# kkromberg/SpeechRecognition

Measured on AMD Instinct MI355X. Metric: frames/sec scored+decoded, higher is better.
Workload: dtype f64

## Files before the change

### include/srgpu.h

```cpp
#ifndef SRGPU_H
#define SRGPU_H

#include <stddef.h>
#include <stdint.h>

#ifdef __cplusplus
extern "C" {
#endif

#if defined(__GNUC__)
#define SR_API __attribute__((visibility("default")))
#else
#define SR_API
#endif

#define SR_ABI_VERSION 4
SR_API int sr_abi_version(void);

#define SR_OK 0
#define SR_EINVAL (-1)
#define SR_EHIP (-2)
#define SR_ENODEV (-3)
#define SR_ELIMIT (-4)
#define SR_ENOMEM (-5)
// ... 252 lines not shown
SR_API int sr_bigram_word_lattice_corpus(sr_model* m, sr_corpus* c, sr_bigram* b, int gmm_kernel, double lattice_beam, uint64_t cap,
                                         uint64_t* out_arc_off, double* out_best, uint32_t* out_word, uint32_t* out_hist,
                                         uint32_t* out_pred, uint32_t* out_first, uint32_t* out_last, double* out_fwd, double* out_bwd,
                                         double* out_am);
SR_API int sr_bigram_lattice_nbest(uint32_t n_frames, uint64_t n_arcs, const uint32_t* word, const uint32_t* hist,
                                   const uint32_t* first, const uint32_t* last, const double* am, uint32_t n_words,
                                   uint32_t silence_word, const float* lm, double lm_scale, uint32_t n_best, uint32_t* out_words,
                                   uint64_t words_cap, uint64_t* out_off, double* out_cost, uint32_t* out_count);

typedef struct sr_bigram_stream sr_bigram_stream;
SR_API int sr_bigram_stream_open(sr_model* m, sr_bigram* b, const sr_bigram_params* p, uint32_t max_streams, uint64_t max_frames,
                                 sr_bigram_stream** out);
SR_API int sr_bigram_stream_begin(sr_bigram_stream* s, uint32_t* id);
SR_API int sr_bigram_stream_push(sr_bigram_stream* s, uint32_t n, const uint32_t* ids, const float* feats, const uint64_t* frame_off);
SR_API int sr_bigram_stream_partial(sr_bigram_stream* s, uint32_t id, uint32_t* out_word, float* out_score, uint32_t* out_time,
                                    uint32_t cap, uint32_t* count, uint64_t* frames);
SR_API int sr_bigram_stream_end(sr_bigram_stream* s, uint32_t id, uint32_t* out_word, float* out_score, uint32_t* out_time,
                                uint32_t cap, uint32_t* count);
SR_API int sr_bigram_stream_destroy(sr_bigram_stream* s);

SR_API int sr_probe_fp16_denormals(int device, int* preserved);
SR_API int sr_probe_fp16_accumulation(int device, int* within_model, double* worst_ratio);

typedef struct {
  double gmm_ms;
  uint64_t gmm_launches;
  double gmm_flops;
  double search_ms;
  uint64_t search_launches;
  double search_bytes;
  uint64_t frames;
  uint64_t refined_pairs;
  uint64_t refined_densities;
  double prefilter_ms;
  double refine_ms;
} sr_profile;
SR_API int sr_profile_enable(sr_model* m, int on);
SR_API int sr_profile_reset(sr_model* m);
SR_API int sr_profile_read(sr_model* m, sr_profile* out);

#ifdef __cplusplus
}
#endif
#endif
```

### speechrecognition_amd/capi.py

```python
from __future__ import annotations

import ctypes as C
import os

import numpy as np

HERE = os.path.dirname(os.path.abspath(__file__))
LIB_PATH = os.environ.get("SRGPU_LIB") or os.path.join(HERE, "libsrgpu.so")

GMM_MFMA, GMM_EXACT, GMM_PREFILTER, GMM_DEFAULT = 0, 1, 2, 3
POOL_GLOBAL, POOL_MIXTURE, POOL_NONE = 0, 1, 2
SEARCH_GENERAL_KERNEL = 1
SEARCH_SLOT_KERNEL = 2
BIGRAM_DENSE_STATES = 1
BIGRAM_GLOBAL_STATES = 2
SR_ECORRUPT = -7
LDA_SKIP = 0xFFFFFFFF
SR_ABI_VERSION = 4

SYMBOLS = [
    "sr_abi_version", "sr_model_trim",
    "sr_last_error", "sr_device_count", "sr_model_create", "sr_model_load_mixset", "sr_model_destroy", "sr_model_info",
    "sr_corpus_upload", "sr_corpus_upload_async", "sr_corpus_wait", "sr_corpus_destroy", "sr_shard_utterances", "sr_recognize_batch_multi", "sr_score_corpus", "sr_score_frames", "sr_lexicon_create",
    "sr_lexicon_destroy", "sr_lexicon_describe", "sr_recognize_corpus", "sr_traceback_corpus", "sr_traceback_words", "sr_recognize_batch", "sr_align_corpus", "sr_align_corpus_pruned", "sr_path_scores_corpus", "sr_model_create_from_statistics", "sr_model_create_from_accumulated", "sr_mixset_write", "sr_model_set_tying", "sr_model_tying_info", "sr_model_topology", "sr_accumulate_corpus",
    "sr_model_split", "sr_model_eliminate", "sr_model_tables",
    "sr_state_posteriors_corpus", "sr_baum_welch_corpus", "sr_word_posteriors_corpus", "sr_recognize_confidence_corpus",
    "sr_net_occupancies_corpus", "sr_mmi_statistics_corpus", "sr_model_create_from_mmi_statistics",
    "sr_smbr_max_positions", "sr_net_accuracies_corpus", "sr_smbr_statistics_corpus",
    "sr_word_lattice_corpus", "sr_lattice_nbest",
    "sr_fmllr_statistics_corpus", "sr_fmllr_statistics_bw_corpus", "sr_fmllr_estimate", "sr_corpus_transform",
    "sr_mllr_statistics_corpus", "sr_mllr_statistics_bw_corpus", "sr_mllr_estimate", "sr_model_transform_means",
    "sr_mllt_statistics_corpus", "sr_mllt_statistics_bw_corpus", "sr_mllt_estimate",
    "sr_lda_statistics_corpus", "sr_lda_estimate", "sr_corpus_splice_transform",
    "sr_bigram_create", "sr_bigram_destroy", "sr_bigram_describe", "sr_recognize_bigram_corpus",
    "sr_bigram_word_posteriors_corpus", "sr_recognize_bigram_confidence_corpus",
    "sr_bigram_occupancies_corpus", "sr_bigram_mmi_statistics_corpus",
    "sr_bigram_accuracies_corpus", "sr_bigram_smbr_statistics_corpus",
    "sr_bigram_word_lattice_corpus", "sr_bigram_lattice_nbest",
    "sr_stream_open", "sr_stream_begin", "sr_stream_push", "sr_stream_partial", "sr_stream_end", "sr_stream_destroy",
    "sr_bigram_stream_open", "sr_bigram_stream_begin", "sr_bigram_stream_push", "sr_bigram_stream_partial", "sr_bigram_stream_end",
    "sr_bigram_stream_destroy",
    "sr_probe_fp16_denormals", "sr_probe_fp16_accumulation",
    "sr_profile_enable", "sr_profile_reset", "sr_profile_read",
]


class SrError(RuntimeError):
    def __init__(self, code, msg):
        super().__init__(f"libsrgpu error {code}: {msg}")
        self.code = code


def smbr_max_positions():
    n = C.c_uint32()
    _check(lib().sr_smbr_max_positions(C.byref(n)))
    return n.value


class SearchParams(C.Structure):
    _fields_ = [("am_threshold", C.c_double), ("word_penalty", C.c_double), ("gmm_kernel", C.c_int), ("flags", C.c_int)]


class BigramParams(C.Structure):
    _fields_ = [("acoustic_pruning", C.c_float), ("lm_pruning", C.c_float), ("gmm_kernel", C.c_int), ("max_word_ends", C.c_uint32), ("flags", C.c_int)]


class Profile(C.Structure):
    _fields_ = [("gmm_ms", C.c_double), ("gmm_launches", C.c_uint64), ("gmm_flops", C.c_double),
                ("search_ms", C.c_double), ("search_launches", C.c_uint64), ("search_bytes", C.c_double),
                ("frames", C.c_uint64), ("refined_pairs", C.c_uint64), ("refined_densities", C.c_uint64),
                ("prefilter_ms", C.c_double), ("refine_ms", C.c_double)]


# ... 77 lines not shown
        L.sr_recognize_bigram_corpus.argtypes = [vp, vp, vp, C.POINTER(BigramParams), vp, vp, vp, vp]
        L.sr_bigram_word_posteriors_corpus.argtypes = [vp, vp, vp, i32, dbl, dbl, u32, vp, vp, vp, vp]
        L.sr_bigram_occupancies_corpus.argtypes = [vp, vp, vp, i32, dbl, dbl, u32, vp, vp, vp, vp, vp, vp]
        L.sr_bigram_mmi_statistics_corpus.argtypes = [vp, vp, vp, i32, dbl, dbl, i32, vp, vp] + [vp] * 10
        L.sr_bigram_accuracies_corpus.argtypes = [vp, vp, vp, i32, dbl, dbl, u32, vp, vp, vp, vp, vp, vp]
        L.sr_bigram_smbr_statistics_corpus.argtypes = [vp, vp, vp, i32, dbl, dbl, i32, vp] + [vp] * 10
        L.sr_recognize_bigram_confidence_corpus.argtypes = [vp, vp, vp, C.POINTER(BigramParams), dbl, vp, vp, vp, vp, vp]
        L.sr_bigram_word_lattice_corpus.argtypes = [vp, vp, vp, i32, dbl, u64] + [vp] * 10
        L.sr_bigram_lattice_nbest.argtypes = [u32, u64, vp, vp, vp, vp, vp, u32, u32, vp, dbl, u32, vp, u64, vp, vp, C.POINTER(u32)]
        L.sr_stream_open.argtypes = [vp, vp, C.POINTER(SearchParams), u32, u64, C.POINTER(vp)]
        L.sr_stream_begin.argtypes = [vp, C.POINTER(u32)]
        L.sr_stream_push.argtypes = [vp, u32, vp, vp, vp]
        L.sr_stream_partial.argtypes = [vp, u32, vp, u32, C.POINTER(u32), C.POINTER(u64)]
        L.sr_stream_end.argtypes = [vp, u32, vp, u32, C.POINTER(u32), vp, vp, vp]
        L.sr_stream_destroy.argtypes = [vp]
        L.sr_bigram_stream_open.argtypes = [vp, vp, C.POINTER(BigramParams), u32, u64, C.POINTER(vp)]
        L.sr_bigram_stream_begin.argtypes = [vp, C.POINTER(u32)]
        L.sr_bigram_stream_push.argtypes = [vp, u32, vp, vp, vp]
        L.sr_bigram_stream_partial.argtypes = [vp, u32, vp, vp, vp, u32, C.POINTER(u32), C.POINTER(u64)]
        L.sr_bigram_stream_end.argtypes = [vp, u32, vp, vp, vp, u32, C.POINTER(u32)]
        L.sr_bigram_stream_destroy.argtypes = [vp]
        L.sr_probe_fp16_denormals.argtypes = [i32, C.POINTER(i32)]
        L.sr_probe_fp16_accumulation.argtypes = [i32, C.POINTER(i32), C.POINTER(dbl)]
        L.sr_profile_enable.argtypes = [vp, i32]
        L.sr_profile_reset.argtypes = [vp]
        L.sr_profile_read.argtypes = [vp, C.POINTER(Profile)]
        _lib = L
    return _lib


def _check(rc):
    if rc != 0:
        raise SrError(rc, lib().sr_last_error().decode(errors="replace"))


def device_count():
    n = C.c_int(0)
    _check(lib().sr_device_count(C.byref(n)))
    return n.value


def _ptr(a):
    return a.ctypes.data if a is not None else None


class Model:
# ... 87 lines not shown
        assert len(cls) == self.n_densities and W.ndim == 3 and W.shape[1:] == (self.dim, self.dim + 1)
        h = C.c_void_p()
        _check(lib().sr_model_transform_means(self.h, _ptr(cls), W.shape[0], _ptr(W), C.byref(h)))
        return Model(h)

    def close(self):
        if self.h:
            lib().sr_model_destroy(self.h)
            self.h = None

    def trim(self):
        _check(lib().sr_model_trim(self.h))

    def __enter__(self):
        return self

    def __exit__(self, *exc):
        self.close()

    def score_frames(self, feats, kernel=GMM_PREFILTER):
        feats = np.ascontiguousarray(feats, dtype=np.float32)
        out = np.empty((feats.shape[0], self.n_states), dtype=np.float64)
        _check(lib().sr_score_frames(self.h, _ptr(feats), feats.shape[0], kernel, _ptr(out)))
        return out

    def upload(self, feats, frame_off, asynchronous=False):
        return Corpus(self, feats, frame_off, asynchronous)

    def recognize_batch(self, lexicon, feats, frame_off, am_threshold, word_penalty, kernel=GMM_PREFILTER):
        feats = np.ascontiguousarray(feats, dtype=np.float32)
        frame_off = np.ascontiguousarray(frame_off, dtype=np.uint64)
        n = len(frame_off) - 1
        words = np.zeros(max(int(frame_off[-1]), 1), dtype=np.uint32)
        woff = np.zeros(n + 1, dtype=np.uint64)
        sp = SearchParams(am_threshold, word_penalty, kernel, 0)
        _check(lib().sr_recognize_batch(self.h, lexicon.h, C.byref(sp), _ptr(feats), _ptr(frame_off), n, _ptr(words), _ptr(woff)))
        return words[: int(woff[-1])].copy(), woff

    def lexicon(self, word_off, automaton, silence_idx, tdp, silence_state):
        return Lexicon(self, word_off, automaton, silence_idx, tdp, silence_state)

    def bigram(self, word_off, mixtures, silence_word, lm, tdp):
        return Bigram(self, word_off, mixtures, silence_word, lm, tdp)

    def stream(self, lexicon, am_threshold, word_penalty, kernel=GMM_PREFILTER, max_streams=1, max_frames=65535):
        return Stream(self, lexicon, am_threshold, word_penalty, kernel, max_streams, max_frames)
# ... 721 lines not shown
```

### speechrecognition_amd/csrc/gmm_prefilter.hip

```cpp
#include <hip/hip_runtime.h>
#include <stdint.h>

#include <algorithm>
#include <cmath>
#include <vector>

#include "kernels.h"

#ifndef SR_P16_NB
#define SR_P16_NB 4
#endif

namespace srgpu {

typedef float v4f __attribute__((ext_vector_type(4)));
static constexpr int kPWaves = 4;
static constexpr int kGroupBlocks = 8;

typedef _Float16 f16x8 __attribute__((ext_vector_type(8)));

__device__ inline uint32_t pack_f16x2(_Float16 l, _Float16 h) {
  return (uint32_t)__builtin_bit_cast(uint16_t, l) | ((uint32_t)__builtin_bit_cast(uint16_t, h) << 16);
}

// ... 138 lines not shown
            : "v"(ap[nb][j][0]), "v"(ap[nb][j][1]), "v"(ap[nb][j][2]), "v"(ap[nb][j][3]), "v"(ap[nb][j + 1][0]),
              "v"(ap[nb][j + 1][1]), "v"(ap[nb][j + 1][2]), "v"(ap[nb][j + 1][3]));
      if (a.chunks >= 2) { const float o = __shfl_xor(amin, 16); asm("v_min_f32 %0, %0, %1" : "+v"(amin) : "v"(o)); }
      if (a.chunks >= 4) { const float o = __shfl_xor(amin, 32); asm("v_min_f32 %0, %0, %1" : "+v"(amin) : "v"(o)); }
      const float limit = amin + __builtin_fmaf(lim.y, dbnorm[nb], __builtin_fmaf(lim.x, bnorm[nb], lim.z));
      uint32_t mask = 0;
#pragma unroll
      for (int j = kGroupBlocks - 1; j >= 1; j -= 2)
        asm("v_cmp_ngt_f32 vcc, %2, %1\n\tv_addc_co_u32 %0, vcc, %0, %0, vcc\n\t"
            "v_cmp_ngt_f32 vcc, %3, %1\n\tv_addc_co_u32 %0, vcc, %0, %0, vcc\n\t"
            "v_cmp_ngt_f32 vcc, %4, %1\n\tv_addc_co_u32 %0, vcc, %0, %0, vcc\n\t"
            "v_cmp_ngt_f32 vcc, %5, %1\n\tv_addc_co_u32 %0, vcc, %0, %0, vcc\n\t"
            "v_cmp_ngt_f32 vcc, %6, %1\n\tv_addc_co_u32 %0, vcc, %0, %0, vcc\n\t"
            "v_cmp_ngt_f32 vcc, %7, %1\n\tv_addc_co_u32 %0, vcc, %0, %0, vcc\n\t"
            "v_cmp_ngt_f32 vcc, %8, %1\n\tv_addc_co_u32 %0, vcc, %0, %0, vcc\n\t"
            "v_cmp_ngt_f32 vcc, %9, %1\n\tv_addc_co_u32 %0, vcc, %0, %0, vcc"
            : "+v"(mask)
            : "v"(limit), "v"(ap[nb][j][3]), "v"(ap[nb][j][2]), "v"(ap[nb][j][1]), "v"(ap[nb][j][0]), "v"(ap[nb][j - 1][3]),
              "v"(ap[nb][j - 1][2]), "v"(ap[nb][j - 1][1]), "v"(ap[nb][j - 1][0])
            : "vcc");
      if (m_ok[nb]) m_ptr[m_off[nb]] = mask;
    }
    m_ptr += a.n_frames * 4u;
  }
}

__global__ void fp16_denormal_probe_kernel(float* out) {
  const int lane = threadIdx.x;
  f16x8 a = {0, 0, 0, 0, 0, 0, 0, 0}, b = {0, 0, 0, 0, 0, 0, 0, 0};
  if (lane < 16) { a[0] = (_Float16)9.5367431640625e-7f; b[0] = (_Float16)1024.0f; }
  v4f acc = {0.f, 0.f, 0.f, 0.f};
  acc = __builtin_amdgcn_mfma_f32_16x16x32_f16(a, b, acc, 0, 0, 0);
  out[lane] = acc[0];
}

hipError_t probe_fp16_denormals(hipStream_t stream, bool* preserved) {
  float* d = nullptr;
  hipError_t e = hipMalloc(reinterpret_cast<void**>(&d), 64 * sizeof(float));
  if (e != hipSuccess) return e;
  hipLaunchKernelGGL(fp16_denormal_probe_kernel, dim3(1), dim3(64), 0, stream, d);
  float h[64];
  e = hipGetLastError();
  if (e == hipSuccess) e = hipStreamSynchronize(stream);
  if (e == hipSuccess) e = hipMemcpy(h, d, sizeof(h), hipMemcpyDeviceToHost);
  (void)hipFree(d);
  if (e != hipSuccess) return e;
// ... 76 lines not shown
  (void)hipFree(dA); (void)hipFree(dB); (void)hipFree(dO);
  if (e != hipSuccess) return e;
  double worst = 0.0;
  bool fine = true;
  for (int t = 0; t < kCases; t++)
    for (int r = 0; r < 16; r++)
      for (int c = 0; c < 16; c++) {
        double exact = 0.0, mag = 0.0;
        for (int k = 0; k < K; k++) {
          const double p = (double)(float)hA[((size_t)t * 16 + r) * K + k] * (double)(float)hB[((size_t)t * K + k) * 16 + c];
          exact += p;
          mag += p < 0 ? -p : p;
        }
        const double err = std::fabs((double)got[(size_t)t * 256 + r * 16 + c] - exact);
        const double ratio = err / (mag * 5.9604644775390625e-8);
        if (!(ratio <= allowed)) fine = false;
        if (ratio > worst || ratio != ratio) worst = ratio;
      }
  *ok = fine;
  if (worst_ratio) *worst_ratio = worst;
  return hipSuccess;
}

hipError_t launch_gmm_prefilter(const GmmPrefilterArgs& a, int ks32, hipStream_t stream) {
  const dim3 grid(a.nx * a.ny), block(kPWaves * 64);
  if (a.n_frames >= (1ull << 30)) return hipErrorInvalidValue;
  switch (ks32) {
    case 1: hipLaunchKernelGGL((gmm_prefilter16_kernel<1, SR_P16_NB>), grid, block, 0, stream, a); break;
    case 2: hipLaunchKernelGGL((gmm_prefilter16_kernel<2, SR_P16_NB>), grid, block, 0, stream, a); break;
    case 3: hipLaunchKernelGGL((gmm_prefilter16_kernel<3, SR_P16_NB>), grid, block, 0, stream, a); break;
    case 4: hipLaunchKernelGGL((gmm_prefilter16_kernel<4, SR_P16_NB>), grid, block, 0, stream, a); break;
    default: return hipErrorInvalidValue;
  }
  return hipGetLastError();
}
int gmm_prefilter_frames_per_tile() { return kPWaves * SR_P16_NB * 16; }

#pragma clang fp contract(off)

#ifndef SR_R_THREADS
#define SR_R_THREADS 768
#endif
#ifndef SR_R_BATCH
#define SR_R_BATCH 4
#endif
static constexpr int kRThreads = SR_R_THREADS;
static constexpr int kRThreadsWide = 512;
static constexpr int kRWaves = kRThreads / 64;
static constexpr int kRBatch = SR_R_BATCH;
// ... 677 lines not shown
```

### speechrecognition_amd/csrc/handles.h

```cpp
#pragma once
#include <hip/hip_runtime.h>

#include <atomic>
#include <condition_variable>
#include <cstdint>
#include <map>
#include <memory>
#include <mutex>
#include <string>
#include <thread>
#include <vector>

#include "../../include/srgpu.h"
#include "host_util.h"
#include "kernels.h"

namespace srhost {
int fail(int code, const char* fmt, ...) __attribute__((format(printf, 2, 3)));
}

#define HIP_TRY(expr)                                                                             \
  do {                                                                                            \
    hipError_t e_ = (expr);                                                                       \
    if (e_ != hipSuccess) return srhost::fail(SR_EHIP, "%s: %s (%s:%d)", #expr, hipGetErrorString(e_), __FILE__, __LINE__); \
// ... 51 lines not shown
  DevBuf<double> means, inv_vars, norm, logw;
  DevBuf<uint32_t> dens_mean, dens_var;
  std::vector<uint32_t> h_dens_off, h_dens_mean, h_dens_var;
  std::vector<double> h_means, h_inv_vars, h_norm, h_logw;
  bool mfma_packed = false, pf_packed = false;
  uint32_t n_mean = 0, n_var = 0;
  int ksteps = 0;
  uint32_t n_blocks = 0, n_groups = 0;
  DevBuf<double> apack;
  DevBuf<uint32_t> blk_meta, grp_state;
  std::vector<uint32_t> group_first_block;
  std::map<uint32_t, std::unique_ptr<DevBuf<uint32_t>>> split_tabs, pf_split_tabs;
  const uint32_t *split_cur = nullptr, *pf_split_cur = nullptr;
  uint32_t split_ny = 0;
  int pf_ks32 = 0;
  uint32_t pf_groups = 0, pf_ny = 0, max_dens = 0, pf_slots = 0, pf_chunks = 1, pf_pstates = 0;
  DevBuf<unsigned char> pf_apack;
  DevBuf<float> pf_lim, featsT, featsP;
  DevBuf<uint4> pf_defer;
  DevBuf<uint32_t> pf_defer_cnt;
  int neg_possible = -1;
  uint32_t pf_dp = 0;
  DevBuf<uint32_t> pf_mask, pf_ndens, pf_ring;
  DevBuf<double> pf_rows;
  DevBuf<unsigned long long> pf_counter;
  hipStream_t s_copy = nullptr;
  float* staging[2] = {nullptr, nullptr};
  hipEvent_t staging_free[2] = {nullptr, nullptr};
  std::atomic<bool> staging_busy{false};
  std::mutex spare_mu;
  std::unique_ptr<CorpusSpare> spare;
  std::vector<sr_corpus*> corpora;
  hipStream_t s_gmm = nullptr, s_search = nullptr;
  DevBuf<double> scores[2];
  hipEvent_t ev_scored[2] = {nullptr, nullptr}, ev_consumed[2] = {nullptr, nullptr};
  size_t chunk_frames = 0;
  bool overlap = true;
  size_t defer_budget = (size_t)32 << 30;
  uint32_t defer_cap_limit = 0;
  size_t fb_budget = (size_t)1 << 30;
  size_t mllt_budget = (size_t)256 << 20;
  size_t lda_budget = (size_t)256 << 20;
  bool profiling = false;
  std::vector<EventPair> events;
  sr_profile prof{};
};
// ... 173 lines not shown
```

### speechrecognition_amd/csrc/kernels.h

```cpp
#pragma once
#include <hip/hip_runtime.h>
#include <stdint.h>

#include <vector>

namespace srgpu {

struct GmmMfmaArgs {
  const float* feats;
  uint64_t n_frames;
  uint32_t dim;
  const double* apack;
  const uint32_t* blk_meta;
  const uint32_t* grp_state;
  const uint32_t* split_begin;
  double* out;
  uint32_t ld;
  uint32_t nx, ny;
};
int gmm_mfma_ksteps_for_dim(uint32_t dim);
int gmm_mfma_frames_per_tile(int ksteps);
hipError_t launch_gmm_mfma(const GmmMfmaArgs& a, int ksteps, bool sum, hipStream_t stream);

struct GmmExactArgs {
// ... 13 lines not shown
hipError_t launch_gmm_exact(const GmmExactArgs& a, bool sum, uint32_t n_splits, hipStream_t stream);
struct GmmExactList {
  const uint64_t* blk_frame0;
  const uint32_t* blk_frames;
  const uint32_t* blk_list;
  const uint32_t* list_off;
  const uint32_t* states;
  uint32_t blk_first;
  uint64_t frame_base;
};
hipError_t launch_gmm_exact_listed(const GmmExactArgs& a, bool sum, const GmmExactList& L, uint32_t n_blocks, hipStream_t stream);
int gmm_exact_frames_per_block();

struct GmmPrefilterArgs {
  const float* feats;
  uint64_t n_frames;
  uint32_t dim;
  const unsigned char* apack;
  const float* grp_lim;
  const uint32_t* split_begin;
  uint32_t* mask;
  uint32_t nx, ny;
  uint32_t chunks;
};
struct PfBound { float kappa, acc, abs, sub; };
constexpr float kPfRes16 = 4.8835e-4f;
inline constexpr PfBound pf_bound(int ks32) {
  return ks32 == 4 ? PfBound{1.05e-3f, 1.6e-5f, 7.0e-7f, 3.38e-7f} : PfBound{1.05e-3f, 1.1e-5f, 6.0e-7f, 2.92e-7f};
}
struct GmmRefineArgs {
  const float* feats;
  const float* featsT;
  uint64_t n_frames, n_frames_ld;
  uint32_t dim, n_pstates, chunks;
  const uint32_t* n_dens_ps;
  const double* rows;
  uint32_t n_slots;
  const uint32_t* mask;
  double* out; uint32_t ld;
  uint64_t frames_per_split;
  unsigned long long* n_refined;
  uint32_t* ring;
  void* defer;
  uint32_t* defer_cnt;
  uint32_t defer_cap;
};
void gmm_refine_defer_layout(const GmmRefineArgs& a, size_t budget_bytes, uint32_t cap_limit, uint32_t* cap, size_t* n_entries,
                             size_t* n_counts);
size_t gmm_refine_ring_words(const GmmRefineArgs& a);
hipError_t launch_gmm_prefilter(const GmmPrefilterArgs& a, int ks32, hipStream_t stream);
int gmm_prefilter_frames_per_tile();
hipError_t probe_fp16_denormals(hipStream_t stream, bool* preserved);
hipError_t probe_fp16_accumulation(hipStream_t stream, int ks32, bool* ok, double* worst_ratio);
uint32_t gmm_refine_padded_dim(uint32_t dim);
int gmm_refine_slots(uint32_t max_dens, uint32_t padded_dim);
hipError_t launch_gmm_refine(const GmmRefineArgs& a, hipStream_t stream);
hipError_t launch_transpose_feats(const float* feats, uint64_t n_frames, uint32_t dim, uint32_t dp, uint64_t ldT, float* out, float* featsP,
                                  hipStream_t stream);

struct DecodeNet {
  uint32_t n_slots;
  uint32_t n_words;
  const uint32_t* slot_info;
  const uint32_t* slot_word;
  const uint32_t* word_end_slot;
  uint32_t silence_word;
  double tdp_loop, tdp_forward, tdp_skip;
  uint32_t silence_state;
};
static constexpr uint32_t kSlotPos0 = 1u << 16;
static constexpr uint32_t kSlotPos1 = 1u << 17;
static constexpr uint32_t kSlotEnd = 1u << 18;
static constexpr uint32_t kSlotSilState = 1u << 19;
static constexpr uint32_t kSlotSilWord = 1u << 20;
// ... 558 lines not shown
```

### speechrecognition_amd/csrc/srgpu_api.cpp

```cpp
#include <hip/hip_runtime.h>

#include <algorithm>
#include <cmath>
#include <cstdarg>
#include <cstdio>
#include <cstdlib>
#include <cstring>
#include <limits>
#include <map>
#include <memory>
#include <mutex>
#include <numeric>
#include <queue>
#include <set>
#include <string>
#include <vector>

#include "../../include/srgpu.h"
#include "fb_plan.h"
#include "host_util.h"
#include "kernels.h"
#include "traceback.h"

using namespace srgpu;
// ... 313 lines not shown
  HIP_TRY(hipEventRecord(ep->b, s));
  m->events.push_back(*ep);
  return SR_OK;
}

int resolve_dense_kernel(const sr_model* m, int gmm_kernel) {
  if (gmm_kernel == SR_GMM_DEFAULT) gmm_kernel = m->max_approx ? SR_GMM_PREFILTER : SR_GMM_MFMA;
  if (gmm_kernel == SR_GMM_MFMA && m->ksteps == 0) gmm_kernel = SR_GMM_EXACT;
  return gmm_kernel;
}

GmmRefineArgs refine_shape(const sr_model* m, uint64_t n_frames) {
  GmmRefineArgs ra{};
  ra.n_frames = n_frames; ra.dim = m->pf_dp; ra.n_pstates = m->pf_pstates; ra.n_slots = m->pf_slots; ra.chunks = m->pf_chunks;
  return ra;
}
struct DeferLayout { uint32_t cap; size_t n_e, n_c; };
DeferLayout defer_layout(const sr_model* m, uint64_t n_frames) {
  DeferLayout d;
  gmm_refine_defer_layout(refine_shape(m, n_frames), m->defer_budget, m->defer_cap_limit, &d.cap, &d.n_e, &d.n_c);
  return d;
}

int reserve_scoring(sr_model* m, int gmm_kernel, uint64_t n_max) {
  gmm_kernel = resolve_dense_kernel(m, gmm_kernel);
  if ((gmm_kernel == SR_GMM_MFMA && !m->mfma_packed) || (gmm_kernel == SR_GMM_PREFILTER && !m->pf_packed)) {
    int rc = srhost::ensure_host_tables(m);
    if (rc) return rc;
  }
  if (gmm_kernel == SR_GMM_MFMA && !m->mfma_packed) {
    int rc = pack_model(m, m->h_dens_off.data(), m->h_means.data(), m->h_inv_vars.data(), m->h_norm.data(), m->h_logw.data());
    if (rc) return rc;
    m->mfma_packed = true;
  }
  if (gmm_kernel == SR_GMM_PREFILTER && !m->pf_packed) {
    int rc = pack_prefilter(m, m->h_dens_off.data(), m->h_means.data(), m->h_inv_vars.data(), m->h_norm.data(), m->h_logw.data());
    if (rc) return rc;
    m->pf_packed = true;
  }
  if (gmm_kernel == SR_GMM_PREFILTER && m->pf_ks32 > 0 && n_max > 0) {
    const uint64_t ldT = (n_max + 63) & ~(uint64_t)63;
    const size_t want_T = (size_t)ldT * m->pf_dp, want_mask = (size_t)((m->pf_groups + 1u) & ~1u) * n_max * 4;
    const size_t want_P = m->pf_dp != m->dim ? (size_t)n_max * m->pf_dp + 4 : 0;
    const size_t want_ring = gmm_refine_ring_words(refine_shape(m, n_max));
    if (want_T > m->featsT.n || want_P > m->featsP.n || want_mask > m->pf_mask.n || want_ring > m->pf_ring.n) HIP_TRY(hipStreamSynchronize(m->s_gmm));
    HIP_TRY(m->featsT.ensure(want_T));
    if (want_P) HIP_TRY(m->featsP.ensure(want_P));
    const DeferLayout dl = defer_layout(m, n_max);
    if (dl.n_e > m->pf_defer.n || dl.n_c > m->pf_defer_cnt.n) HIP_TRY(hipStreamSynchronize(m->s_gmm));
    if (dl.n_e) { HIP_TRY(m->pf_defer.ensure(dl.n_e)); HIP_TRY(m->pf_defer_cnt.ensure(dl.n_c)); }
    HIP_TRY(m->pf_mask.ensure(want_mask));
    HIP_TRY(m->pf_ring.ensure(want_ring));
  }
  return SR_OK;
}

int launch_scoring(sr_model* m, const float* d_feats, uint64_t n_frames, int gmm_kernel, double* d_out) {
  if (n_frames == 0) return SR_OK;
  gmm_kernel = resolve_dense_kernel(m, gmm_kernel);
  EventPair ep{};
  {
    int rc = reserve_scoring(m, gmm_kernel, n_frames);
    if (rc) return rc;
  }
  if (gmm_kernel == SR_GMM_MFMA) {
    const uint32_t tile = gmm_mfma_frames_per_tile(m->ksteps);
    const uint32_t nx = (uint32_t)((n_frames + tile - 1) / tile);
    int rc = set_splits(m, nx);
    if (rc) return rc;
    GmmMfmaArgs a{};
    a.feats = d_feats; a.n_frames = n_frames; a.dim = m->dim;
    a.apack = m->apack.p; a.blk_meta = m->blk_meta.p; a.grp_state = m->grp_state.p; a.split_begin = m->split_cur;
    a.out = d_out; a.ld = m->ld; a.nx = nx; a.ny = m->split_ny;
    if ((rc = prof_begin(m, m->s_gmm, 0, &ep))) return rc;
    HIP_TRY(launch_gmm_mfma(a, m->ksteps, !m->max_approx, m->s_gmm));
    if ((rc = prof_end(m, m->s_gmm, &ep))) return rc;
  } else if (gmm_kernel == SR_GMM_PREFILTER && m->pf_ks32 > 0) {
    const uint32_t tile = gmm_prefilter_frames_per_tile();
    const uint32_t nx = (uint32_t)((n_frames + tile - 1) / tile);
    int rc = set_prefilter_splits(m, nx);
    if (rc) return rc;
    const uint64_t ldT = (n_frames + 63) & ~(uint64_t)63;
    GmmPrefilterArgs pa{};
    pa.feats = d_feats; pa.n_frames = n_frames; pa.dim = m->dim;
    pa.apack = m->pf_apack.p; pa.grp_lim = m->pf_lim.p; pa.split_begin = m->pf_split_cur;
    pa.mask = m->pf_mask.p; pa.nx = nx; pa.ny = m->pf_ny; pa.chunks = std::min(4u, m->pf_chunks);
    GmmRefineArgs ra = refine_shape(m, n_frames);
    const bool padded = m->pf_dp != m->dim;
    ra.feats = padded ? m->featsP.p : d_feats; ra.featsT = m->featsT.p; ra.n_frames_ld = ldT;
    ra.n_dens_ps = m->pf_ndens.p; ra.rows = m->pf_rows.p;
    ra.mask = m->pf_mask.p; ra.out = d_out; ra.ld = m->ld;
    ra.n_refined = m->profiling ? m->pf_counter.p : nullptr;
    ra.ring = m->pf_ring.p;
    const DeferLayout dl = defer_layout(m, n_frames);
    if (dl.cap && dl.n_e <= m->pf_defer.n && dl.n_c <= m->pf_defer_cnt.n) { ra.defer = m->pf_defer.p; ra.defer_cnt = m->pf_defer_cnt.p; ra.defer_cap = dl.cap; }
    if (m->profiling) m->prof.refined_pairs += n_frames * (uint64_t)m->n_states;
    EventPair ep_p{}, ep_r{};
    if ((rc = prof_begin(m, m->s_gmm, 0, &ep))) return rc;
    if ((rc = prof_begin(m, m->s_gmm, 2, &ep_p))) return rc;
    HIP_TRY(launch_transpose_feats(d_feats, n_frames, m->dim, m->pf_dp, ldT, m->featsT.p, padded ? m->featsP.p : nullptr, m->s_gmm));
    HIP_TRY(launch_gmm_prefilter(pa, m->pf_ks32, m->s_gmm));
    if ((rc = prof_end(m, m->s_gmm, &ep_p))) return rc;
    if ((rc = prof_begin(m, m->s_gmm, 3, &ep_r))) return rc;
    HIP_TRY(launch_gmm_refine(ra, m->s_gmm));
    if ((rc = prof_end(m, m->s_gmm, &ep_r))) return rc;
    if ((rc = prof_end(m, m->s_gmm, &ep))) return rc;
  } else if (gmm_kernel == SR_GMM_EXACT || gmm_kernel == SR_GMM_PREFILTER) {
    GmmExactArgs a{};
    a.feats = d_feats; a.n_frames = n_frames; a.dim = m->dim; a.n_states = m->n_states;
    a.dens_off = m->dens_off.p; a.means = m->means.p; a.inv_vars = m->inv_vars.p; a.norm = m->norm.p; a.logw = m->logw.p;
    a.out = d_out; a.ld = m->ld;
    const uint32_t nx = (uint32_t)((n_frames + 255) / 256);
    uint32_t ny = std::max(1u, std::min(m->n_states, (4096 + nx - 1) / nx));
    a.states_per_split = (m->n_states + ny - 1) / ny;
    ny = (m->n_states + a.states_per_split - 1) / a.states_per_split;
    int rc;
    if ((rc = prof_begin(m, m->s_gmm, 0, &ep))) return rc;
    HIP_TRY(launch_gmm_exact(a, !m->max_approx, ny, m->s_gmm));
    if ((rc = prof_end(m, m->s_gmm, &ep))) return rc;
  } else {
    return fail(SR_EINVAL, "unknown gmm_kernel %d", gmm_kernel);
  }
  if (m->profiling) m->prof.gmm_flops += 4.0 * m->dim * (double)m->n_dens * (double)n_frames;
  return SR_OK;
// ... 240 lines not shown
  hipError_t e;
  if ((e = hipStreamCreateWithFlags(&m->s_gmm, hipStreamNonBlocking)) != hipSuccess ||
      (e = hipStreamCreateWithFlags(&m->s_search, hipStreamNonBlocking)) != hipSuccess)
    return fail(SR_EHIP, "hipStreamCreate: %s", hipGetErrorString(e));
  for (int i = 0; i < 2; i++)
    if ((e = hipEventCreateWithFlags(&m->ev_scored[i], hipEventDisableTiming)) != hipSuccess ||
        (e = hipEventCreateWithFlags(&m->ev_consumed[i], hipEventDisableTiming)) != hipSuccess)
      return fail(SR_EHIP, "hipEventCreate: %s", hipGetErrorString(e));
  if ((e = m->dens_off.upload(dens_off, n_states + 1)) != hipSuccess) return fail(SR_EHIP, "model upload: %s", hipGetErrorString(e));
  uint32_t mx = 0;
  for (uint32_t s = 0; s < n_states; s++) mx = std::max(mx, dens_off[s + 1] - dens_off[s]);
  m->max_dens = std::max(1u, mx);
  m->h_dens_off.assign(dens_off, dens_off + n_states + 1);
  const char* env = getenv("SRGPU_SCORE_CHUNK_MB");
  size_t chunk_bytes = (size_t)49152 << 20;
  {
    size_t free_b = 0, total_b = 0;
    if (hipMemGetInfo(&free_b, &total_b) == hipSuccess && total_b) chunk_bytes = std::min(chunk_bytes, total_b / 6);
  }
  if (env) chunk_bytes = (size_t)atol(env) << 20;
  m->chunk_frames = std::max<size_t>(1, chunk_bytes / ((size_t)m->ld * sizeof(double)));
  m->chunk_frames = std::min<size_t>(m->chunk_frames, ((size_t)1 << 32) / (4 * (size_t)dim) - 128);
  if (const char* ov = getenv("SRGPU_OVERLAP")) m->overlap = atoi(ov) != 0;
  if (const char* e = getenv("SRGPU_DEFER_MB")) m->defer_budget = (size_t)strtoull(e, nullptr, 10) << 20;
  if (const char* e = getenv("SRGPU_FB_MB")) m->fb_budget = std::max<size_t>(1, (size_t)strtoull(e, nullptr, 10)) << 20;
  if (const char* e = getenv("SRGPU_MLLT_MB")) m->mllt_budget = std::max<size_t>(1, (size_t)strtoull(e, nullptr, 10)) << 20;
  if (const char* e = getenv("SRGPU_LDA_MB")) m->lda_budget = std::max<size_t>(1, (size_t)strtoull(e, nullptr, 10)) << 20;
  if (const char* e = getenv("SRGPU_DEFER_CAP")) m->defer_cap_limit = std::max(1u, (uint32_t)strtoul(e, nullptr, 10));
  *out = own.release();
  return SR_OK;
}

int ensure_host_tables(sr_model* m) {
  const size_t C = m->n_dens, D = m->dim;
  if (m->h_norm.size() == C && m->h_means.size() == C * D) return SR_OK;
  m->h_means.resize(C * D); m->h_inv_vars.resize(C * D); m->h_norm.resize(C); m->h_logw.resize(C);
  if (C == 0) return SR_OK;
  HIP_TRY(hipMemcpy(m->h_means.data(), m->means.p, C * D * sizeof(double), hipMemcpyDeviceToHost));
  HIP_TRY(hipMemcpy(m->h_inv_vars.data(), m->inv_vars.p, C * D * sizeof(double), hipMemcpyDeviceToHost));
  HIP_TRY(hipMemcpy(m->h_norm.data(), m->norm.p, C * sizeof(double), hipMemcpyDeviceToHost));
  HIP_TRY(hipMemcpy(m->h_logw.data(), m->logw.p, C * sizeof(double), hipMemcpyDeviceToHost));
  return SR_OK;
}

int may_go_negative(sr_model* m, bool* out) {
  if (m->neg_possible < 0) {
// ... 180 lines not shown
  }
  if (m->profiling) m->prof.frames += F;
  return SR_OK;
  });
}

int sr_score_frames(sr_model* m, const float* feats, uint64_t n_frames, int gmm_kernel, double* out) {
  return guarded(__func__, [&]() -> int {
  const uint64_t off[2] = {0, n_frames};
  int rc = check_model(m);
  if (rc) return rc;
  if (n_frames > 0 && (!feats || !out)) return fail(SR_EINVAL, "%s is null", feats ? "out" : "feats");
  if (n_frames > (std::numeric_limits<size_t>::max() / sizeof(float) - 64) / m->dim)
    return fail(SR_ELIMIT, "n_frames %llu x dim %u overflows the address space", (unsigned long long)n_frames, m->dim);
  sr_corpus* c = new sr_corpus();
  std::unique_ptr<sr_corpus, int (*)(sr_corpus*)> own(c, sr_corpus_destroy);
  c->model = m; c->n_utts = 1; c->n_frames = n_frames; c->frame_off.assign(off, off + 2);
  srhost::corpus_register(c);
  hipError_t e;
  if ((e = c->feats.ensure((size_t)n_frames * m->dim + 64)) != hipSuccess ||
      (n_frames > 0 && (e = hipMemcpy(c->feats.p, feats, (size_t)n_frames * m->dim * sizeof(float), hipMemcpyHostToDevice)) != hipSuccess))
    return fail(SR_EHIP, "feature upload: %s", hipGetErrorString(e));
  return sr_score_corpus(m, c, gmm_kernel, out);
  });
}

int sr_lexicon_create(sr_model* m, uint32_t n_words, const uint32_t* word_off, const uint16_t* automaton,
                      uint32_t silence_idx, const double tdp[3], uint16_t silence_state, sr_lexicon** out) {
  return guarded(__func__, [&]() -> int {
  if (!out) return fail(SR_EINVAL, "out is null");
  *out = nullptr;
  int rc = check_model(m);
  if (rc) return rc;
  if (!word_off || !automaton || !tdp) return fail(SR_EINVAL, "null lexicon table");
  if (n_words == 0 || n_words > 65535) return fail(SR_ELIMIT, "n_words must be 1..65535 (Book::word is 16 bit)");
  if (silence_idx >= n_words) return fail(SR_EINVAL, "silence_idx out of range");
  if (word_off[0] != 0) return fail(SR_EINVAL, "word_off[0] must be 0");
  uint32_t max_pos = 0;
  for (uint32_t w = 0; w < n_words; w++) {
    if (word_off[w + 1] <= word_off[w]) return fail(SR_EINVAL, "word %u has no positions", w);
    max_pos = std::max(max_pos, word_off[w + 1] - word_off[w]);
  }
  if (max_pos < 2) return fail(SR_ELIMIT, "lexicon needs at least one word with two or more positions");
  const uint32_t P = word_off[n_words];
  if (P > decode_big_max_slots()) return fail(SR_ELIMIT, "%u trellis positions exceed the decoder's limit of %u", P, decode_big_max_slots());
  for (uint32_t w = 0; w < n_words; w++)
// ... 3360 lines not shown
```

Measured before the change: 13.43 million.

## Add stationary-weights GMM prefilter route with precomputed fp16 feature fragments

Adds a new default prefilter route. A first kernel converts the features once into fp16 MFMA B-fragments plus per-frame norms. A second kernel then keeps each group's packed density operands resident in registers while it streams frame ranges, with a double-buffered fetch, and writes the masks. Work is split across XCD-interleaved workgroups using a plan that maximises grid fill. The intent is to stop reloading weights and recomputing the feature conversion per tile, at the cost of an extra launch, extra device buffers, and high register pressure.

```diff
diff --git a/include/srgpu.h b/include/srgpu.h
--- a/include/srgpu.h
+++ b/include/srgpu.h
@@ -298,6 +298,10 @@
 SR_API int sr_probe_fp16_denormals(int device, int* preserved);
 SR_API int sr_probe_fp16_accumulation(int device, int* within_model, double* worst_ratio);
 
+SR_API int sr_prefilter_masks(sr_model* m, const float* feats, uint64_t n_frames, int route, uint32_t* n_groups, uint32_t* masks,
+                              uint64_t cap_words);
+SR_API int sr_prefilter_range_frames(uint32_t* frames);
+
 typedef struct {
   double gmm_ms;
   uint64_t gmm_launches;
diff --git a/speechrecognition_amd/capi.py b/speechrecognition_amd/capi.py
--- a/speechrecognition_amd/capi.py
+++ b/speechrecognition_amd/capi.py
@@ -40,7 +40,7 @@
     "sr_stream_open", "sr_stream_begin", "sr_stream_push", "sr_stream_partial", "sr_stream_end", "sr_stream_destroy",
     "sr_bigram_stream_open", "sr_bigram_stream_begin", "sr_bigram_stream_push", "sr_bigram_stream_partial", "sr_bigram_stream_end",
     "sr_bigram_stream_destroy",
-    "sr_probe_fp16_denormals", "sr_probe_fp16_accumulation",
+    "sr_probe_fp16_denormals", "sr_probe_fp16_accumulation", "sr_prefilter_masks", "sr_prefilter_range_frames",
     "sr_profile_enable", "sr_profile_reset", "sr_profile_read",
 ]
 
@@ -49,6 +49,12 @@
     def __init__(self, code, msg):
         super().__init__(f"libsrgpu error {code}: {msg}")
         self.code = code
+
+
+def prefilter_range_frames():
+    n = C.c_uint32()
+    _check(lib().sr_prefilter_range_frames(C.byref(n)))
+    return n.value
 
 
 def smbr_max_positions():
@@ -172,6 +178,8 @@
         L.sr_bigram_stream_destroy.argtypes = [vp]
         L.sr_probe_fp16_denormals.argtypes = [i32, C.POINTER(i32)]
         L.sr_probe_fp16_accumulation.argtypes = [i32, C.POINTER(i32), C.POINTER(dbl)]
+        L.sr_prefilter_masks.argtypes = [vp, vp, u64, i32, C.POINTER(u32), vp, u64]
+        L.sr_prefilter_range_frames.argtypes = [C.POINTER(u32)]
         L.sr_profile_enable.argtypes = [vp, i32]
         L.sr_profile_reset.argtypes = [vp]
         L.sr_profile_read.argtypes = [vp, C.POINTER(Profile)]
@@ -305,6 +313,14 @@
         feats = np.ascontiguousarray(feats, dtype=np.float32)
         out = np.empty((feats.shape[0], self.n_states), dtype=np.float64)
         _check(lib().sr_score_frames(self.h, _ptr(feats), feats.shape[0], kernel, _ptr(out)))
+        return out
+
+    def prefilter_masks(self, feats, route):
+        feats = np.ascontiguousarray(feats, dtype=np.float32)
+        n_groups = C.c_uint32()
+        _check(lib().sr_prefilter_masks(self.h, None, feats.shape[0], route, C.byref(n_groups), None, 0))
+        out = np.empty((n_groups.value, feats.shape[0], 4), dtype=np.uint32)
+        _check(lib().sr_prefilter_masks(self.h, _ptr(feats), feats.shape[0], route, C.byref(n_groups), _ptr(out), out.size))
         return out
 
     def upload(self, feats, frame_off, asynchronous=False):
diff --git a/speechrecognition_amd/csrc/gmm_prefilter.hip b/speechrecognition_amd/csrc/gmm_prefilter.hip
--- a/speechrecognition_amd/csrc/gmm_prefilter.hip
+++ b/speechrecognition_amd/csrc/gmm_prefilter.hip
@@ -184,6 +184,156 @@
       if (m_ok[nb]) m_ptr[m_off[nb]] = mask;
     }
     m_ptr += a.n_frames * 4u;
+  }
+}
+
+#ifndef SR_PS_PIN
+#define SR_PS_PIN 1
+#endif
+#if SR_PS_PIN
+#define SR_PS_PIN_FETCH __builtin_amdgcn_sched_barrier(0)
+#else
+#define SR_PS_PIN_FETCH (void)0
+#endif
+static constexpr int kSNB = 2;
+static constexpr int kSRangeFrames = 2048;
+
+template <int KS32>
+__global__ __launch_bounds__(kPWaves * 64) void gmm_prefilter_operands_kernel(const float* feats, uint64_t n_frames, uint32_t dim,
+                                                                              uint64_t n_blocks, uint4* bfrag, float2* bnorm) {
+  const int lane = threadIdx.x & 63, wave = threadIdx.x >> 6;
+  const uint32_t g = lane >> 4, c = lane & 15;
+  const uint64_t blk = (uint64_t)blockIdx.x * kPWaves + wave;
+  if (blk >= n_blocks) return;
+  const uint64_t f = blk * 16 + c;
+  const bool valid = f < n_frames;
+  const float* xr = feats + (valid ? f : 0u) * dim;
+  float n2 = 0.0f, e2 = 0.0f;
+#pragma unroll
+  for (int ks = 0; ks < KS32; ks++) {
+    _Float16 v[8];
+#pragma unroll
+    for (int j = 0; j < 8; j++) {
+      const uint32_t k = 32u * ks + 8u * g + j, d = k >> 1;
+      const float xf = (valid && d < dim) ? xr[d < dim ? d : 0u] : 0.0f;
+      const float b = (k & 1u) ? xf : xf * xf;
+      n2 += b * b;
+      _Float16 h = (_Float16)b;
+      const float bh = (float)h;
+      const float e = (k & 1u) ? xf - bh : __builtin_fmaf(xf, xf, -bh);
+      e2 += e * e;
+      if (valid && k >= 2u * dim && k < 2u * dim + 3u) h = (_Float16)1.0f;
+      v[j] = h;
+    }
+    bfrag[(blk * KS32 + ks) * 64 + lane] =
+        make_uint4(pack_f16x2(v[0], v[1]), pack_f16x2(v[2], v[3]), pack_f16x2(v[4], v[5]), pack_f16x2(v[6], v[7]));
+  }
+  n2 += __shfl_xor(n2, 16);
+  n2 += __shfl_xor(n2, 32);
+  e2 += __shfl_xor(e2, 16);
+  e2 += __shfl_xor(e2, 32);
+  const float bn = sqrtf(n2) * 1.0001f;
+  const float dbn = fminf(sqrtf(e2) * 1.0001f, kPfRes16 * bn);
+  if (g == 0) bnorm[f] = make_float2(bn, dbn);
+}
+
+struct GmmStationaryPlan { uint32_t n_quads, n_ranges, range_frames, per_xcd; };
+
+template <int KS32>
+__global__ __launch_bounds__(kPWaves * 64, 2) void gmm_prefilter_stationary_kernel(GmmPrefilterArgs a, GmmStationaryPlan p) {
+  constexpr int NB = kSNB;
+  constexpr int kGroupBytes = kGroupBlocks * KS32 * 1024;
+  const int lane = threadIdx.x & 63, wave = threadIdx.x >> 6;
+  const int g = lane >> 4, c = lane & 15;
+  const uint32_t item = (blockIdx.x & 7u) * p.per_xcd + (blockIdx.x >> 3);
+  if ((blockIdx.x >> 3) >= p.per_xcd || item >= p.n_quads * p.n_ranges) return;
+  const uint32_t grp = (item % p.n_quads) * kPWaves + wave;
+  if (grp >= a.n_groups) return;
+  const uint64_t f_begin = (uint64_t)(item / p.n_quads) * p.range_frames;
+  if (f_begin >= a.n_frames) return;
+  const uint64_t f_end = f_begin + p.range_frames < a.n_frames ? f_begin + p.range_frames : a.n_frames;
+  const uint32_t n_steps = (uint32_t)((f_end - f_begin + 16 * NB - 1) / (16 * NB));
+
+  f16x8 af[kGroupBlocks][KS32];
+  {
+    const uint4* src = reinterpret_cast<const uint4*>(a.apack + (uint64_t)grp * kGroupBytes) + lane;
+#pragma unroll
+    for (int j = 0; j < kGroupBlocks; j++)
+#pragma unroll
+      for (int ks = 0; ks < KS32; ks++) af[j][ks] = __builtin_bit_cast(f16x8, src[(j * KS32 + ks) * 64]);
+  }
+  const float4 lim = reinterpret_cast<const float4*>(a.grp_lim)[4u * grp + g];
+
+  const uint4* b_src = a.bfrag + (f_begin / 16) * (KS32 * 64) + lane;
+  const float2* n_src = a.bnorm + f_begin + c;
+  uint32_t* m_ptr = a.mask + (uint64_t)grp * a.n_frames * 4u;
+  uint4 bq[2][NB][KS32];
+  float2 nq[2][NB];
+  auto fetch = [&](int buf, uint32_t s) __attribute__((always_inline)) {
+    const uint4* bs = b_src + (uint64_t)s * (NB * KS32 * 64);
+#pragma unroll
+    for (int nb = 0; nb < NB; nb++) {
+#pragma unroll
+      for (int ks = 0; ks < KS32; ks++) bq[buf][nb][ks] = bs[(nb * KS32 + ks) * 64];
+      nq[buf][nb] = n_src[(uint64_t)s * (NB * 16) + nb * 16];
+    }
+  };
+  auto step = [&](int buf, uint32_t s) __attribute__((always_inline)) {
+    v4f ap[NB][kGroupBlocks];
+#pragma unroll
+    for (int nb = 0; nb < NB; nb++)
+#pragma unroll
+      for (int j = 0; j < kGroupBlocks; j++) ap[nb][j] = (v4f){0.f, 0.f, 0.f, 0.f};
+#pragma unroll
+    for (int ks = 0; ks < KS32; ks++)
+#pragma unroll
+      for (int j = 0; j < kGroupBlocks; j++)
+#pragma unroll
+        for (int nb = 0; nb < NB; nb++)
+          ap[nb][j] = __builtin_amdgcn_mfma_f32_16x16x32_f16(af[j][ks], __builtin_bit_cast(f16x8, bq[buf][nb][ks]), ap[nb][j], 0, 0, 0);
+    __builtin_amdgcn_sched_barrier(0);
+    asm volatile("s_nop 7");
+    __builtin_amdgcn_sched_barrier(0);
+#pragma unroll
+    for (int nb = 0; nb < NB; nb++) {
+      float amin = __builtin_huge_valf();
+#pragma unroll
+      for (int j = 0; j < kGroupBlocks; j += 2)
+        asm("v_min3_f32 %0, %0, %1, %2\n\tv_min3_f32 %0, %0, %3, %4\n\tv_min3_f32 %0, %0, %5, %6\n\tv_min3_f32 %0, %0, %7, %8"
+            : "+v"(amin)
+            : "v"(ap[nb][j][0]), "v"(ap[nb][j][1]), "v"(ap[nb][j][2]), "v"(ap[nb][j][3]), "v"(ap[nb][j + 1][0]),
+              "v"(ap[nb][j + 1][1]), "v"(ap[nb][j + 1][2]), "v"(ap[nb][j + 1][3]));
+      if (a.chunks >= 2) { const float o = __shfl_xor(amin, 16); asm("v_min_f32 %0, %0, %1" : "+v"(amin) : "v"(o)); }
+      if (a.chunks >= 4) { const float o = __shfl_xor(amin, 32); asm("v_min_f32 %0, %0, %1" : "+v"(amin) : "v"(o)); }
+      const float limit = amin + __builtin_fmaf(lim.y, nq[buf][nb].y, __builtin_fmaf(lim.x, nq[buf][nb].x, lim.z));
+      uint32_t mask = 0;
+#pragma unroll
+      for (int j = kGroupBlocks - 1; j >= 1; j -= 2)
+        asm("v_cmp_ngt_f32 vcc, %2, %1\n\tv_addc_co_u32 %0, vcc, %0, %0, vcc\n\t"
+            "v_cmp_ngt_f32 vcc, %3, %1\n\tv_addc_co_u32 %0, vcc, %0, %0, vcc\n\t"
+            "v_cmp_ngt_f32 vcc, %4, %1\n\tv_addc_co_u32 %0, vcc, %0, %0, vcc\n\t"
+            "v_cmp_ngt_f32 vcc, %5, %1\n\tv_addc_co_u32 %0, vcc, %0, %0, vcc\n\t"
+            "v_cmp_ngt_f32 vcc, %6, %1\n\tv_addc_co_u32 %0, vcc, %0, %0, vcc\n\t"
+            "v_cmp_ngt_f32 vcc, %7, %1\n\tv_addc_co_u32 %0, vcc, %0, %0, vcc\n\t"
+            "v_cmp_ngt_f32 vcc, %8, %1\n\tv_addc_co_u32 %0, vcc, %0, %0, vcc\n\t"
+            "v_cmp_ngt_f32 vcc, %9, %1\n\tv_addc_co_u32 %0, vcc, %0, %0, vcc"
+            : "+v"(mask)
+            : "v"(limit), "v"(ap[nb][j][3]), "v"(ap[nb][j][2]), "v"(ap[nb][j][1]), "v"(ap[nb][j][0]), "v"(ap[nb][j - 1][3]),
+              "v"(ap[nb][j - 1][2]), "v"(ap[nb][j - 1][1]), "v"(ap[nb][j - 1][0])
+            : "vcc");
+      const uint64_t f = f_begin + (uint64_t)s * (NB * 16) + nb * 16 + c;
+      if (f < a.n_frames) m_ptr[(uint32_t)f * 4u + (uint32_t)g] = mask;
+    }
+  };
+  fetch(0, 0);
+  for (uint32_t s = 0; s < n_steps; s += 2) {
+    fetch(1, s + 1 < n_steps ? s + 1 : n_steps - 1);
+    SR_PS_PIN_FETCH;
+    step(0, s);
+    if (s + 1 >= n_steps) break;
+    fetch(0, s + 2 < n_steps ? s + 2 : n_steps - 1);
+    SR_PS_PIN_FETCH;
+    step(1, s + 1);
   }
 }
 
@@ -306,9 +456,59 @@
   return hipSuccess;
 }
 
-hipError_t launch_gmm_prefilter(const GmmPrefilterArgs& a, int ks32, hipStream_t stream) {
+static GmmStationaryPlan stationary_plan(uint32_t n_groups, uint64_t n_frames) {
+  GmmStationaryPlan p{};
+  p.n_quads = (n_groups + kPWaves - 1) / kPWaves;
+  const uint64_t steps = (n_frames + 16 * kSNB - 1) / (16 * kSNB);
+  const uint64_t r_max = std::max<uint64_t>(1, std::min<uint64_t>(steps, (n_frames + kSRangeFrames - 1) / kSRangeFrames));
+  uint64_t best_r = 1;
+  double best = -1.0;
+  for (uint64_t r = 1; r <= r_max; r++) {
+    const uint64_t wgs = (uint64_t)p.n_quads * r;
+    const double fill = (double)wgs / (double)((wgs + 511) / 512 * 512);
+    if (fill > best * (1.0 + 1e-9)) { best = fill; best_r = r; }
+  }
+  const uint64_t range_steps = (steps + best_r - 1) / best_r;
+  p.range_frames = (uint32_t)(range_steps * 16 * kSNB);
+  p.n_ranges = (uint32_t)((steps + range_steps - 1) / range_steps);
+  p.per_xcd = (uint32_t)(((uint64_t)p.n_quads * p.n_ranges + 7) / 8);
+  return p;
+}
+
+int gmm_prefilter_route(int ks32, int route) { return (route == kPfStationary && ks32 >= 1 && ks32 <= 3) ? kPfStationary : kPfStaged; }
+int gmm_prefilter_stationary_range_frames() { return kSRangeFrames; }
+void gmm_prefilter_operand_sizes(int ks32, uint64_t n_frames, size_t* n_frag, size_t* n_norm) {
+  const uint64_t blocks = (n_frames + 16 * kSNB - 1) / (16 * kSNB) * kSNB;
+  *n_frag = (size_t)blocks * ks32 * 64;
+  *n_norm = (size_t)blocks * 16;
+}
+
+template <int KS32>
+static hipError_t launch_stationary(const GmmPrefilterArgs& a, hipStream_t stream) {
+  if (!a.bfrag || !a.bnorm || a.n_groups == 0) return hipErrorInvalidValue;
+  size_t n_frag, n_norm;
+  gmm_prefilter_operand_sizes(KS32, a.n_frames, &n_frag, &n_norm);
+  const uint64_t blocks = n_norm / 16;
+  hipLaunchKernelGGL((gmm_prefilter_operands_kernel<KS32>), dim3((unsigned)((blocks + kPWaves - 1) / kPWaves)), dim3(kPWaves * 64), 0, stream,
+                     a.feats, a.n_frames, a.dim, blocks, a.bfrag, a.bnorm);
+  hipError_t e = hipGetLastError();
+  if (e != hipSuccess) return e;
+  const GmmStationaryPlan p = stationary_plan(a.n_groups, a.n_frames);
+  hipLaunchKernelGGL((gmm_prefilter_stationary_kernel<KS32>), dim3(8 * p.per_xcd), dim3(kPWaves * 64), 0, stream, a, p);
+  return hipGetLastError();
+}
+
+hipError_t launch_gmm_prefilter(const GmmPrefilterArgs& a, int ks32, int route, hipStream_t stream) {
+  if (a.n_frames >= (1ull << 30)) return hipErrorInvalidValue;
+  if (a.n_frames == 0) return hipSuccess;
+  if (gmm_prefilter_route(ks32, route) == kPfStationary) {
+    switch (ks32) {
+      case 1: return launch_stationary<1>(a, stream);
+      case 2: return launch_stationary<2>(a, stream);
+      default: return launch_stationary<3>(a, stream);
+    }
+  }
   const dim3 grid(a.nx * a.ny), block(kPWaves * 64);
-  if (a.n_frames >= (1ull << 30)) return hipErrorInvalidValue;
   switch (ks32) {
     case 1: hipLaunchKernelGGL((gmm_prefilter16_kernel<1, SR_P16_NB>), grid, block, 0, stream, a); break;
     case 2: hipLaunchKernelGGL((gmm_prefilter16_kernel<2, SR_P16_NB>), grid, block, 0, stream, a); break;
diff --git a/speechrecognition_amd/csrc/handles.h b/speechrecognition_amd/csrc/handles.h
--- a/speechrecognition_amd/csrc/handles.h
+++ b/speechrecognition_amd/csrc/handles.h
@@ -97,6 +97,9 @@
   int neg_possible = -1;
   uint32_t pf_dp = 0;
   DevBuf<uint32_t> pf_mask, pf_ndens, pf_ring;
+  DevBuf<uint4> pf_bfrag;
+  DevBuf<float2> pf_bnorm;
+  int pf_route = srgpu::kPfStationary;
   DevBuf<double> pf_rows;
   DevBuf<unsigned long long> pf_counter;
   hipStream_t s_copy = nullptr;
diff --git a/speechrecognition_amd/csrc/kernels.h b/speechrecognition_amd/csrc/kernels.h
--- a/speechrecognition_amd/csrc/kernels.h
+++ b/speechrecognition_amd/csrc/kernels.h
@@ -59,7 +59,11 @@
   uint32_t* mask;
   uint32_t nx, ny;
   uint32_t chunks;
-};
+  uint32_t n_groups;
+  uint4* bfrag;
+  float2* bnorm;
+};
+enum { kPfStaged = 0, kPfStationary = 1 };
 struct PfBound { float kappa, acc, abs, sub; };
 constexpr float kPfRes16 = 4.8835e-4f;
 inline constexpr PfBound pf_bound(int ks32) {
@@ -85,8 +89,11 @@
 void gmm_refine_defer_layout(const GmmRefineArgs& a, size_t budget_bytes, uint32_t cap_limit, uint32_t* cap, size_t* n_entries,
                              size_t* n_counts);
 size_t gmm_refine_ring_words(const GmmRefineArgs& a);
-hipError_t launch_gmm_prefilter(const GmmPrefilterArgs& a, int ks32, hipStream_t stream);
+hipError_t launch_gmm_prefilter(const GmmPrefilterArgs& a, int ks32, int route, hipStream_t stream);
+int gmm_prefilter_route(int ks32, int route);
 int gmm_prefilter_frames_per_tile();
+int gmm_prefilter_stationary_range_frames();
+void gmm_prefilter_operand_sizes(int ks32, uint64_t n_frames, size_t* n_frag, size_t* n_norm);
 hipError_t probe_fp16_denormals(hipStream_t stream, bool* preserved);
 hipError_t probe_fp16_accumulation(hipStream_t stream, int ks32, bool* ok, double* worst_ratio);
 uint32_t gmm_refine_padded_dim(uint32_t dim);
diff --git a/speechrecognition_amd/csrc/srgpu_api.cpp b/speechrecognition_amd/csrc/srgpu_api.cpp
--- a/speechrecognition_amd/csrc/srgpu_api.cpp
+++ b/speechrecognition_amd/csrc/srgpu_api.cpp
@@ -359,8 +359,9 @@
   return d;
 }
 
-int reserve_scoring(sr_model* m, int gmm_kernel, uint64_t n_max) {
+int reserve_scoring(sr_model* m, int gmm_kernel, uint64_t n_max, int pf_route = -1) {
   gmm_kernel = resolve_dense_kernel(m, gmm_kernel);
+  if (pf_route < 0) pf_route = m->pf_route;
   if ((gmm_kernel == SR_GMM_MFMA && !m->mfma_packed) || (gmm_kernel == SR_GMM_PREFILTER && !m->pf_packed)) {
     int rc = srhost::ensure_host_tables(m);
     if (rc) return rc;
@@ -388,7 +389,26 @@
     if (dl.n_e) { HIP_TRY(m->pf_defer.ensure(dl.n_e)); HIP_TRY(m->pf_defer_cnt.ensure(dl.n_c)); }
     HIP_TRY(m->pf_mask.ensure(want_mask));
     HIP_TRY(m->pf_ring.ensure(want_ring));
-  }
+    if (gmm_prefilter_route(m->pf_ks32, pf_route) == kPfStationary) {
+      size_t want_frag, want_norm;
+      gmm_prefilter_operand_sizes(m->pf_ks32, n_max, &want_frag, &want_norm);
+      if (want_frag > m->pf_bfrag.n || want_norm > m->pf_bnorm.n) HIP_TRY(hipStreamSynchronize(m->s_gmm));
+      HIP_TRY(m->pf_bfrag.ensure(want_frag));
+      HIP_TRY(m->pf_bnorm.ensure(want_norm));
+    }
+  }
+  return SR_OK;
+}
+
+int prefilter_args(sr_model* m, const float* d_feats, uint64_t n_frames, GmmPrefilterArgs* pa) {
+  const uint32_t tile = gmm_prefilter_frames_per_tile();
+  const uint32_t nx = (uint32_t)((n_frames + tile - 1) / tile);
+  int rc = set_prefilter_splits(m, nx);
+  if (rc) return rc;
+  pa->feats = d_feats; pa->n_frames = n_frames; pa->dim = m->dim;
+  pa->apack = m->pf_apack.p; pa->grp_lim = m->pf_lim.p; pa->split_begin = m->pf_split_cur;
+  pa->mask = m->pf_mask.p; pa->nx = nx; pa->ny = m->pf_ny; pa->chunks = std::min(4u, m->pf_chunks);
+  pa->n_groups = m->pf_groups; pa->bfrag = m->pf_bfrag.p; pa->bnorm = m->pf_bnorm.p;
   return SR_OK;
 }
 
@@ -413,15 +433,10 @@
     HIP_TRY(launch_gmm_mfma(a, m->ksteps, !m->max_approx, m->s_gmm));
     if ((rc = prof_end(m, m->s_gmm, &ep))) return rc;
   } else if (gmm_kernel == SR_GMM_PREFILTER && m->pf_ks32 > 0) {
-    const uint32_t tile = gmm_prefilter_frames_per_tile();
-    const uint32_t nx = (uint32_t)((n_frames + tile - 1) / tile);
-    int rc = set_prefilter_splits(m, nx);
+    GmmPrefilterArgs pa{};
+    int rc = prefilter_args(m, d_feats, n_frames, &pa);
     if (rc) return rc;
     const uint64_t ldT = (n_frames + 63) & ~(uint64_t)63;
-    GmmPrefilterArgs pa{};
-    pa.feats = d_feats; pa.n_frames = n_frames; pa.dim = m->dim;
-    pa.apack = m->pf_apack.p; pa.grp_lim = m->pf_lim.p; pa.split_begin = m->pf_split_cur;
-    pa.mask = m->pf_mask.p; pa.nx = nx; pa.ny = m->pf_ny; pa.chunks = std::min(4u, m->pf_chunks);
     GmmRefineArgs ra = refine_shape(m, n_frames);
     const bool padded = m->pf_dp != m->dim;
     ra.feats = padded ? m->featsP.p : d_feats; ra.featsT = m->featsT.p; ra.n_frames_ld = ldT;
@@ -436,7 +451,7 @@
     if ((rc = prof_begin(m, m->s_gmm, 0, &ep))) return rc;
     if ((rc = prof_begin(m, m->s_gmm, 2, &ep_p))) return rc;
     HIP_TRY(launch_transpose_feats(d_feats, n_frames, m->dim, m->pf_dp, ldT, m->featsT.p, padded ? m->featsP.p : nullptr, m->s_gmm));
-    HIP_TRY(launch_gmm_prefilter(pa, m->pf_ks32, m->s_gmm));
+    HIP_TRY(launch_gmm_prefilter(pa, m->pf_ks32, m->pf_route, m->s_gmm));
     if ((rc = prof_end(m, m->s_gmm, &ep_p))) return rc;
     if ((rc = prof_begin(m, m->s_gmm, 3, &ep_r))) return rc;
     HIP_TRY(launch_gmm_refine(ra, m->s_gmm));
@@ -723,6 +738,11 @@
   m->chunk_frames = std::max<size_t>(1, chunk_bytes / ((size_t)m->ld * sizeof(double)));
   m->chunk_frames = std::min<size_t>(m->chunk_frames, ((size_t)1 << 32) / (4 * (size_t)dim) - 128);
   if (const char* ov = getenv("SRGPU_OVERLAP")) m->overlap = atoi(ov) != 0;
+  if (const char* e = getenv("SRGPU_PREFILTER")) {
+    if (!strcmp(e, "staged")) m->pf_route = kPfStaged;
+    else if (!strcmp(e, "stationary")) m->pf_route = kPfStationary;
+    else return fail(SR_EINVAL, "SRGPU_PREFILTER=%s: staged or stationary", e);
+  }
   if (const char* e = getenv("SRGPU_DEFER_MB")) m->defer_budget = (size_t)strtoull(e, nullptr, 10) << 20;
   if (const char* e = getenv("SRGPU_FB_MB")) m->fb_budget = std::max<size_t>(1, (size_t)strtoull(e, nullptr, 10)) << 20;
   if (const char* e = getenv("SRGPU_MLLT_MB")) m->mllt_budget = std::max<size_t>(1, (size_t)strtoull(e, nullptr, 10)) << 20;
@@ -949,6 +969,40 @@
       (n_frames > 0 && (e = hipMemcpy(c->feats.p, feats, (size_t)n_frames * m->dim * sizeof(float), hipMemcpyHostToDevice)) != hipSuccess))
     return fail(SR_EHIP, "feature upload: %s", hipGetErrorString(e));
   return sr_score_corpus(m, c, gmm_kernel, out);
+  });
+}
+
+int sr_prefilter_masks(sr_model* m, const float* feats, uint64_t n_frames, int route, uint32_t* n_groups, uint32_t* masks, uint64_t cap_words) {
+  return guarded(__func__, [&]() -> int {
+  int rc = check_model(m);
+  if (rc) return rc;
+  if (route != kPfStaged && route != kPfStationary) return fail(SR_EINVAL, "route %d: 0 (staged) or 1 (stationary)", route);
+  if (!m->max_approx) return fail(SR_EINVAL, "the prefilter scores max-approx models only");
+  if ((rc = reserve_scoring(m, SR_GMM_PREFILTER, n_frames, route))) return rc;
+  if (m->pf_ks32 == 0) return fail(SR_EINVAL, "this model is not scored through the prefilter");
+  if (n_groups) *n_groups = m->pf_groups;
+  if (!masks || n_frames == 0) return SR_OK;
+  if (!feats) return fail(SR_EINVAL, "feats is null");
+  const uint64_t words = (uint64_t)m->pf_groups * n_frames * 4;
+  if (cap_words < words) return fail(SR_EINVAL, "masks holds %llu words, %llu needed", (unsigned long long)cap_words, (unsigned long long)words);
+  DevBuf<float> d_feats;
+  HIP_TRY(d_feats.ensure((size_t)n_frames * m->dim + 64));
+  HIP_TRY(hipMemcpy(d_feats.p, feats, (size_t)n_frames * m->dim * sizeof(float), hipMemcpyHostToDevice));
+  GmmPrefilterArgs pa{};
+  if ((rc = prefilter_args(m, d_feats.p, n_frames, &pa))) return rc;
+  HIP_TRY(hipMemsetAsync(m->pf_mask.p, 0xA5, words * sizeof(uint32_t), m->s_gmm));
+  HIP_TRY(launch_gmm_prefilter(pa, m->pf_ks32, route, m->s_gmm));
+  HIP_TRY(hipStreamSynchronize(m->s_gmm));
+  HIP_TRY(hipMemcpy(masks, m->pf_mask.p, words * sizeof(uint32_t), hipMemcpyDeviceToHost));
+  return SR_OK;
+  });
+}
+
+int sr_prefilter_range_frames(uint32_t* frames) {
+  return guarded(__func__, [&]() -> int {
+  if (!frames) return fail(SR_EINVAL, "frames is null");
+  *frames = (uint32_t)gmm_prefilter_stationary_range_frames();
+  return SR_OK;
   });
 }
 
```

Measured after the change: 13.65 million, median of 6. 1.7% higher.
